# Jianxff/svo_pro_universal

Hardware: AMD Instinct MI355X
Metric: aligned patches/sec + ms/frame, EuRoC 640x480 mono, 1/2/4/8 MI355X (higher is better)
Workload: dtype f64

## Files before the change

### svo_pro_universal_amd/csrc/sparse_align.hip

```cpp
#include <atomic>
#include <cstdlib>
#include <cstring>

#include <type_traits>

#include "svoh_internal.h"
#include "svoh_device_utils.h"
#include "svoh_math.h"

#define SVOH_ALIGN_DRAIN(ctx) SVOH_HIP_TRY(ctx, svoh::align_drain(ctx))

namespace svoh {

static hipError_t align_drain(svoh_ctx* ctx);

static hipError_t align_side_setup(svoh_ctx* ctx, void* h, void* d, size_t bytes)
{
  if (ctx->align_copy_stream) return hipSuccess;
  hipError_t e = ctx->align_launches_since_drain ? align_drain(ctx) : hipSuccess;
  hipEvent_t* evs[] = { &ctx->ev_align_kernel[0], &ctx->ev_align_kernel[1], &ctx->ev_align_uploaded, &ctx->ev_align_delivered };
  for (hipEvent_t* ev : evs)
    if (e == hipSuccess && !*ev) e = hipEventCreateWithFlags(ev, hipEventDisableTiming);
  if (e == hipSuccess) e = hipStreamCreateWithFlags(&ctx->align_copy_stream, hipStreamNonBlocking);
  if (bytes > ((size_t)1 << 20)) bytes = (size_t)1 << 20;
// ... 59 lines not shown
  int32_t n_features;
  int32_t feat_off;
};

struct DevProblemDesc {
  int32_t n_cams, cam_begin;
  svoh_se3 T_init;
  double alpha_init, beta_init;
  svoh_align_prior prior;
};

struct AlignKernelArgs {
  const DevProblemDesc* problems;
  const DevCamDesc* cams;
  svoh_align_result* results;
  double* wpk;
  int64_t slots;
  uint8_t* wsel;
  uint8_t* wvis;
  svoh_align_options opt;
  int32_t lds_img_bytes;
  int32_t rig_build;
  int32_t latency_build;
  int32_t lds_two_per_cu;
  int32_t ws_lds_bytes;
  int32_t eval_level;
  double* eval_out;
  long long* stamps;
  int32_t n_problems;
  int32_t* queue;
  int32_t one_each;
  const svoh_align_gn_state* ext_state;
  int32_t raw_sums;
  int32_t cluster;
  double* xchg;
  unsigned int* bar;
#ifdef SVOH_TEST_HOOKS
  int32_t cluster_test_absent;
#endif
};

constexpr int kXchgStride = 64;

#ifdef SVOH_PHASE_STAMPS
#define SVOH_STAMP_DECL long long st_t0 = 0, st_acc[8] = {0, 0, 0, 0, 0, 0, 0, 0}; const long long st_begin = (long long)__builtin_amdgcn_s_memtime();
#define SVOH_STAMP_START() do { st_t0 = (long long)__builtin_amdgcn_s_memtime(); } while (0)
#define SVOH_STAMP_ADD(k) do { long long st_n = (long long)__builtin_amdgcn_s_memtime(); st_acc[k] += st_n - st_t0; st_t0 = st_n; } while (0)
// ... 146 lines not shown
    const ImgView<RLDS>& ref, const ImgView<CLDS>& cur, int ru, int rv, double rsu, double rsv, int cu, int cv,
    double csu, double csv, double one_plus_alpha, double beta, bool robust, float weight_scale,
    double (&mom)[AccLayout<D>::NMOM])
{
  constexpr int P = PW;
  constexpr int WB = P + 2;
  const double rwtl = (1.0 - rsu) * (1.0 - rsv), rwtr = rsu * (1.0 - rsv);
  const double rwbl = (1.0 - rsu) * rsv, rwbr = rsu * rsv;
  const double cwtl = ((1.0 - csu) * (1.0 - csv)) * one_plus_alpha, cwtr = (csu * (1.0 - csv)) * one_plus_alpha;
  const double cwbl = ((1.0 - csu) * csv) * one_plus_alpha, cwbr = (csu * csv) * one_plus_alpha;

  const int roff = rv * ref.pitch + ru;
  const int coff = cv * cur.pitch + cu;
  if constexpr (ZERO) {
#pragma unroll
    for (int k = 0; k < AccLayout<D>::NMOM; ++k) mom[k] = 0.0;
  }

  unsigned rawA[WB + 1], rawB[WB + 1];
  double it0[WB], it1[WB], it2[WB];
  unsigned curA[P + 1], curB[P + 1];
  PackedRow<WB + 1> pref_r;
  PackedRow<P + 1> pref_c;
  if constexpr (!RLDS) {
    PackedRow<WB + 1> r0, r1, r2;
    ref.template fetch<WB + 1>(roff, r0);
    ref.template fetch<WB + 1>(roff + ref.pitch, r1);
    ref.template fetch<WB + 1>(roff + 2 * ref.pitch, r2);
    ref.template fetch<WB + 1>(roff + 3 * ref.pitch, pref_r);
    if constexpr (!CLDS) {
      PackedRow<P + 1> c0;
      cur.template fetch<P + 1>(coff, c0);
      cur.template fetch<P + 1>(coff + cur.pitch, pref_c);
      ImgView<false>::unpack<P + 1>(c0, curB);
    }
    ImgView<false>::unpack<WB + 1>(r0, rawA);
    ImgView<false>::unpack<WB + 1>(r1, rawB);
#pragma unroll
    for (int i = 0; i < WB; ++i)
      it1[i] = rwtl * (double)rawA[i] + rwtr * (double)rawA[i + 1] + rwbl * (double)rawB[i] + rwbr * (double)rawB[i + 1];
    ImgView<false>::unpack<WB + 1>(r2, rawA);
  } else {
    ref.template row<WB + 1>(roff, rawA);
    ref.template row<WB + 1>(roff + ref.pitch, rawB);
#pragma unroll
    for (int i = 0; i < WB; ++i)
      it1[i] = rwtl * (double)rawA[i] + rwtr * (double)rawA[i + 1] + rwbl * (double)rawB[i] + rwbr * (double)rawB[i + 1];
    ref.template row<WB + 1>(roff + 2 * ref.pitch, rawA);
  }
#pragma unroll
  for (int i = 0; i < WB; ++i)
    it2[i] = rwtl * (double)rawB[i] + rwtr * (double)rawB[i + 1] + rwbl * (double)rawA[i] + rwbr * (double)rawA[i + 1];
  if constexpr (RLDS || CLDS) cur.template row<P + 1>(coff, curB);

  constexpr int kRowUnroll = GONLY ? 4 : (ROB ? 1 : (PH == 8 ? 4 : (D == 8 ? 1 : 2)));
#pragma unroll kRowUnroll
  for (int y = 0; y < PH; ++y) {
    const int rrow = roff + (y + 3) * ref.pitch;
    const int crow = coff + (y + 1) * cur.pitch;
#pragma unroll
    for (int i = 0; i < P + 1; ++i) curA[i] = curB[i];
    if constexpr (!RLDS && !CLDS) {
      ImgView<false>::unpack<WB + 1>(pref_r, rawB);
      ImgView<false>::unpack<P + 1>(pref_c, curB);
      if (y + 1 < PH) {
        ref.template fetch<WB + 1>(rrow + ref.pitch, pref_r);
        cur.template fetch<P + 1>(crow + cur.pitch, pref_c);
      }
      asm volatile("" ::: "memory");
    } else {
      ref.template row<WB + 1>(rrow, rawB);
      cur.template row<P + 1>(crow, curB);
    }
#pragma unroll
    for (int i = 0; i < WB; ++i) {
      it0[i] = it1[i];
      it1[i] = it2[i];
      it2[i] = rwtl * (double)rawA[i] + rwtr * (double)rawA[i + 1] + rwbl * (double)rawB[i] +
               rwbr * (double)rawB[i + 1];
    }
#pragma unroll
    for (int i = 0; i < WB + 1; ++i) rawA[i] = rawB[i];
#pragma unroll
    for (int x = 0; x < P; ++x) {
      const double ref_val = it1[x + 1];
      const double dx = it1[x + 2] - it1[x];
      const double dy = it2[x + 1] - it0[x + 1];
      const double res = fma(cwtl, (double)curA[x], fma(cwtr, (double)curA[x + 1], fma(cwbl, (double)curB[x], fma(cwbr, (double)curB[x + 1], beta - ref_val))));
      if constexpr (GONLY) {
        mom[3] += dx * res;
        mom[4] += dy * res;
        mom[5] += res * res;
// ... 373 lines not shown
    const double ru_tl = zu.y * scale - patch_center_wb;
    const double rv_tl = vs.x * scale - patch_center_wb;
    const int ru = (int)floor(ru_tl), rv = (int)floor(rv_tl);
    const double rsu = ru_tl - ru, rsv = rv_tl - rv;
    double mom[AccLayout<D>::NMOM];
    patch_rows_moments<P, LPP, D, LDS, LDS, GONLY, ROB>(ref, cur, ru, rv, rsu, rsv, cu, cv, csu, csv, r, one_plus_alpha, beta_d, robust,
                                                   weight_scale, mom);
#pragma unroll
    for (int k = 0; k < AccLayout<D>::NMOM; ++k)
      if (!GONLY || k == 3 || k == 4 || k == 5 || k == 13 || k == 14) asm volatile("" : "+v"(mom[k]));
    SVOH_PASS_STAMP(3);
    double ja[6], jb[6];
    jac_rows(jc, cm, dist_jac, X, scale, ja, jb);
    if constexpr (GONLY) accumulate_patch_gradient<D>(mom, ja, jb, est_alpha, est_beta, acc);
    else accumulate_patch<D>(mom, ja, jb, est_alpha, est_beta, acc);
#ifdef SVOH_PHASE_STAMPS
    asm volatile("" : "+v"(acc[0]), "+v"(acc[1]), "+v"(acc[2]));
#endif
    SVOH_PASS_STAMP(4);
  }
}

constexpr int kStageDoubles = 2 * kWsPairs * 128;
template <int P, int D, int NT, bool LDS, bool GONLY = false, bool ROB = false>
__device__ __forceinline__ void accumulate_camera_staged(
    const AlignKernelArgs& a, const CamPass& cd, const ImgView<LDS>& ref, const ImgView<LDS>& cur, int cw, int ch,
    const Rigid& Tcr, double scale, double one_plus_alpha, double beta_d, bool est_alpha, bool est_beta,
    bool robust, bool dist_jac, float weight_scale, int tid, double* stage, const double* jc,
    double (&acc)[GONLY ? D + 1 : AccLayout<D>::NACC], int& nvis, int& changed, int stride = NT)
{
  typedef const __attribute__((address_space(1))) void* gptr;
  typedef __attribute__((address_space(3))) void* lptr;
  const CamModel cm = load_camera(cd.cam);
  const double patch_center = (P - 1) / 2.0f;
  const double patch_center_wb = (P + 2 - 1) / 2.0f;
  const int lane = tid & 63;
  const int n = cd.n_features;
  const int n_round = (n + stride - 1) / stride * stride;
  auto request = [&](double* buf, int64_t gi) {
#pragma unroll
    for (int pr = 0; pr < kWsPairs; ++pr)
      __builtin_amdgcn_global_load_lds((gptr)ws_pair(a, pr, gi), (lptr)(buf + pr * 128), 16, 0, 0);
  };
  if (tid < n) request(stage, cd.feat_off + tid);
  int which = 0;
  for (int i = tid; i < n_round; i += stride, which ^= 1) {
    const int64_t gi = cd.feat_off + i;
    const bool in_range = i < n;
    double* buf = stage + which * (kWsPairs * 128);
// ... 15 lines not shown
        double u, v;
        project3(cm, Y, u, v);
        const double u_tl = u * scale - patch_center;
        const double v_tl = v * scale - patch_center;
        vis = !(u_tl < 0.0 || v_tl < 0.0 || u_tl + P + 2.0 >= cw || v_tl + P + 2.0 >= ch);
        vis = vis && u_tl == u_tl && v_tl == v_tl;
        if (vis) {
          const double fu = floor(u_tl), fv = floor(v_tl);
          cu = (int)fu; cv = (int)fv;
          csu = u_tl - cu; csv = v_tl - cv;
        }
      }
      if constexpr (GONLY) changed |= (int)((vs.y == 2.0) != vis);
      else {
        ws_pair(a, 2, gi)[1] = vis ? 2.0 : 1.0;
        if (a.eval_level >= 0) a.wvis[gi] = vis ? 1 : 0;
      }
      if (vis) {
        ++nvis;
        const double ru_tl = zu.y * scale - patch_center_wb;
        const double rv_tl = vs.x * scale - patch_center_wb;
        const int ru = (int)floor(ru_tl), rv = (int)floor(rv_tl);
        const double rsu = ru_tl - ru, rsv = rv_tl - rv;
        patch_moments<P, D, LDS, LDS, GONLY, ROB>(ref, cur, ru, rv, rsu, rsv, cu, cv, csu, csv, one_plus_alpha, beta_d,
                                                  robust, weight_scale, mom);
      }
    }
    if (vis) {
      if constexpr (LDS) {
#pragma unroll
        for (int k = 0; k < AccLayout<D>::NMOM; ++k)
          if (!GONLY || k == 3 || k == 4 || k == 5 || k == 13 || k == 14) asm volatile("" : "+v"(mom[k]));
      }

      asm volatile("" ::: "memory");
      const double2 xy2 = *reinterpret_cast<const double2*>(buf + 0 * 128 + lane * 2);
      const double z2 = buf[1 * 128 + lane * 2];
      const Vec3 X = { xy2.x, xy2.y, z2 };
      double ja[6], jb[6];
      jac_rows(jc, cm, dist_jac, X, scale, ja, jb);
      if constexpr (GONLY) accumulate_patch_gradient<D>(mom, ja, jb, est_alpha, est_beta, acc);
      else accumulate_patch<D>(mom, ja, jb, est_alpha, est_beta, acc);
    }
    __builtin_amdgcn_s_waitcnt(0xC07F);
  }
}

template <int NT>
__device__ __forceinline__ bool cluster_sum(const AlignKernelArgs& a, int prob, int share, unsigned& epoch, double* vals, int n,
                                            int tid, int* s_flag)
{
  const int G = a.cluster;
// ... 309 lines not shown
      s.Told = T; s.alpha_old = alpha; s.beta_old = beta;
      s.T = Tn; s.alpha = an; s.beta = bn;
      if (level_done) s.level_done = 1;
    }
    T = Tn; alpha = an; beta = bn;
  }
  SVOH_WAVE_STAMP(2);
  {
    const int c = lane < n_cams ? lane : 0;
    const Rigid Tcr = mul(mul(s.cam_cur_T_cam_imu[c], T), s.cam_ref_T_imu_cam[c]);
    if (lane < n_cams) s.Tcr[c] = Tcr;
    if (lane == 0) { s.alpha_f = (float)alpha; s.beta_f = (float)beta; }
  }
  SVOH_WAVE_STAMP(3);
}

template <int P, int NT, bool ILLUM, bool CLUSTER = false, bool ROBUST = false, int LPP = 1, bool LAT = false, bool RIG = false>
__global__ __launch_bounds__(NT, (NT == 256 ? (LAT ? 1 : 2) : 2))
void sparse_align_kernel(const AlignKernelArgs a)
{
  static_assert(!LAT || (NT == 256 && !CLUSTER && LPP == 1), "latency build: the 256-thread lane-per-patch geometry");
  static_assert(!RIG || (!CLUSTER && LPP == 1 && (LAT || NT == 512)), "rig build: the two lane-per-patch geometries of small launches");
  static_assert(LPP == 1 || (!CLUSTER && NT == 512 && LPP <= P), "rows geometry: 512 threads, no cluster mode");
  static_assert(NT == 256 || NT == 512, "workgroups of 256 or 512 threads");
  constexpr bool ROWS = LPP > 1;
  constexpr int D = ILLUM ? 8 : 6;
  constexpr int NACC = AccLayout<D>::NACC;
  constexpr int NW = NT / 64;

  constexpr bool STAGED = NT == 256 && !ROWS;
  constexpr bool kStageRegs = NT == 256 && !LAT && !CLUSTER && !ROWS;
  extern __shared__ __align__(16) unsigned char lds_img[];
  __shared__ __align__(16) double s_stage[STAGED ? NW * kStageDoubles : 2];
  __shared__ double s_jc[SVOH_MAX_CAMS][kJacConsts];
  __shared__ int s_lvl_off[SVOH_MAX_LEVELS];
  __shared__ double s_red[NW][NACC];
  static_assert(NACC <= 45, "g_sum is sized for the 8-parameter case");
  __shared__ double s_x[kXchgStride];
  __shared__ int s_cluster_ok;

  const int tid = threadIdx.x;
  const int lane = tid & 63, wave = tid >> 6;
  __shared__ int s_pbi;
  __shared__ StageItem s_stage_items[kMaxStageItems];
  for (;;) {
  __syncthreads();
  if (tid == 0) s_pbi = atomicAdd(a.queue, 1);
  __syncthreads();
  const int pbi = s_pbi;
  if (pbi >= a.n_problems) break;
#ifdef SVOH_TEST_HOOKS
  if (CLUSTER && a.cluster_test_absent && pbi % a.cluster == 1) continue;
#endif
  const DevProblemDesc& pb = a.problems[pbi];
// ... 103 lines not shown
      if (n_local * kWsPairs * 16 <= a.ws_lds_bytes) {
        ws.base = reinterpret_cast<double*>(lds_img + a.lds_img_bytes);
        ws.slots = n_local;
        ws.first = cams[0].feat_off;
      }
    }
  }
  {
    int my_sel = 0;
    const int patch_size_wb = P + 2;
    const double scale = 1.0f / (1 << opt.max_level);
    const double patch_center_wb = (patch_size_wb - 1) / 2.0f;
    for (int c = 0; c < n_cams; ++c) {
      const DevCamDesc& cd = cams[c];
      const int rows_minus_two = cd.ref[opt.max_level].h - 2;
      const int cols_minus_two = cd.ref[opt.max_level].w - 2;
      struct FeatIn { double pu, pv, pwx, pwy, pwz, fx, fy, fz; unsigned flag; };
      auto request = [&](int k, FeatIn& o) {
        o.flag = cd.flags[k];
        o.pu = cd.px[2 * k]; o.pv = cd.px[2 * k + 1];
        o.pwx = cd.pos_world[3 * k + 0]; o.pwy = cd.pos_world[3 * k + 1]; o.pwz = cd.pos_world[3 * k + 2];
        o.fx = cd.f[3 * k + 0]; o.fy = cd.f[3 * k + 1]; o.fz = cd.f[3 * k + 2];
      };
      constexpr int kBaseDepth = 4;
      for (int i0 = tid; i0 < cd.n_features; i0 += kBaseDepth * NT) {
        FeatIn in[kBaseDepth];
#pragma unroll
        for (int k = 0; k < kBaseDepth; ++k) {
          in[k] = FeatIn{ 0, 0, 0, 0, 0, 0, 0, 0, 0u };
          if (i0 + k * NT < cd.n_features) request(i0 + k * NT, in[k]);
        }
#pragma unroll
        for (int k = 0; k < kBaseDepth; ++k) {
          const int i = i0 + k * NT;
          if (i >= cd.n_features) break;
          const int gi = cd.feat_off + i;
          bool sel = in[k].flag != 0;
          const double pu = in[k].pu, pv = in[k].pv;
          const double pwx = in[k].pwx, pwy = in[k].pwy, pwz = in[k].pwz;
          const double fx_ = in[k].fx, fy_ = in[k].fy, fz_ = in[k].fz;
          if (sel) {
            const double u_tl = pu * scale - patch_center_wb;
            const double v_tl = pv * scale - patch_center_wb;
            const int u_tl_i = (int)floor(u_tl);
            const int v_tl_i = (int)floor(v_tl);
            sel = !(u_tl_i < 0 || v_tl_i < 0 || u_tl_i >= cols_minus_two - patch_size_wb ||
                    v_tl_i >= rows_minus_two - patch_size_wb);
          }
          a.wsel[gi] = sel ? 1 : 0;
          a.wvis[gi] = 0;
          if (!sel) *reinterpret_cast<double2*>(ws_pair(ws, 2, gi)) = make_double2(0.0, 0.0);
          if (sel) {
            const double dx = pwx - cd.ref_pos[0];
            const double dy = pwy - cd.ref_pos[1];
            const double dz = pwz - cd.ref_pos[2];
            const double depth = sqrt(dx * dx + dy * dy + dz * dz);
            const Vec3 X = { fx_ * depth, fy_ * depth, fz_ * depth };
            *reinterpret_cast<double2*>(ws_pair(ws, 0, gi)) = make_double2(X.x, X.y);
            *reinterpret_cast<double2*>(ws_pair(ws, 1, gi)) = make_double2(X.z, pu);
            *reinterpret_cast<double2*>(ws_pair(ws, 2, gi)) = make_double2(pv, 1.0);
            ++my_sel;
          }
        }
      }
    }
    if (my_sel) atomicAdd(&g_state.nsel, my_sel);
  }
  __syncthreads();
  SVOH_STAMP_ADD(0);
  constexpr bool cluster = CLUSTER;
  const int c_prob = cluster ? pbi / a.cluster : pbi;
  const int c_share = cluster ? pbi % a.cluster : 0;
  const int res_idx = cluster ? (c_share == 0 ? c_prob : a.n_problems / a.cluster + pbi) : pbi;
// ... 24 lines not shown
  const bool est_alpha = opt.estimate_illumination_gain != 0;
  const bool est_beta = opt.estimate_illumination_offset != 0;
  constexpr bool robust = ROBUST;
  const bool dist_jac = opt.use_distortion_jacobian != 0;
  const float weight_scale = (float)opt.weight_scale;

  constexpr int kLanesPerPatch = ROWS ? LPP : 1;
  bool side_by_side = false;
  if (RIG && n_cams >= 2) {
    int lanes_needed = 0;
    for (int c = 0; c < n_cams; ++c) lanes_needed += (cams[c].n_features * kLanesPerPatch + 63) & ~63;
    side_by_side = lanes_needed <= NT;
  }

  for (int level = level_hi; level >= level_lo; --level) {
    const double scale = 1.0f / (1 << level);
    int lvl_off = s_lvl_off[level];
    bool in_lds = lvl_off >= 0;
    if (!in_lds && level_bytes(level) <= a.lds_img_bytes) {
      __syncthreads();
      stage_level(level, 0);
      lvl_off = 0;
      in_lds = true;
    }
    __builtin_amdgcn_s_waitcnt(0x0F70);
    __syncthreads();
    if (tid == 0) {
      g_state.level_done = 0;
      for (int c = 0; c < n_cams; ++c)
        g_state.Tcr[c] = mul(mul(g_state.cam_cur_T_cam_imu[c], g_state.T), g_state.cam_ref_T_imu_cam[c]);
      g_state.alpha_f = (float)g_state.alpha; g_state.beta_f = (float)g_state.beta;
      g_state.Told = g_state.T; g_state.alpha_old = g_state.alpha; g_state.beta_old = g_state.beta;
    }
    __syncthreads();
    SVOH_STAMP_ADD(1);

    for (int iter = 0; iter < opt.max_iter; ++iter) {
      const double one_plus_alpha = uniform_f64(1.0 + (double)g_state.alpha_f);
      const double beta_d = uniform_f64((double)g_state.beta_f);
      bool light = !eval_mode && !robust && iter > 0;
      for (;;) {
        int nvis = 0, changed = 0;
        auto run_cameras = [&](auto gonly_tag, auto& acc_ref) {
          constexpr bool G = decltype(gonly_tag)::value;
          int off = lvl_off;
          int cam_base = 0;
          for (int c = 0; c < n_cams; ++c) {
            const DevCamDesc& cdg = cams[c];
            CamPass cd;
            cd.cam = cdg.cam; cd.n_features = cdg.n_features; cd.feat_off = cdg.feat_off;
            const DevImage& rim = cdg.ref[level];
            const DevImage& cim = cdg.cur[level];
            const Rigid Tcr = uniform_rigid(g_state.Tcr[c]);
            unsigned cam_stride = NT, cam_t = (unsigned)tid;
            if (RIG && side_by_side) {
              const int cam_width = (cd.n_features * kLanesPerPatch + 63) & ~63;
              cam_stride = (unsigned)cam_width;
              cam_t = (unsigned)(tid - cam_base);
              cam_base += cam_width;
            }
            if (in_lds) {
              ImgView<true> ref, cur;
              ref.p = (const __attribute__((address_space(3))) uint8_t*)(lds_img + off); ref.pitch = rim.w;
              off += ((rim.w * rim.h + 15) & ~15);
              cur.p = (const __attribute__((address_space(3))) uint8_t*)(lds_img + off); cur.pitch = cim.w;
              off += ((cim.w * cim.h + 15) & ~15);
              if constexpr (ROWS) {
                if (!RIG || cam_t < cam_stride)
                  accumulate_camera_rows<P, (ROWS ? LPP : 2), D, NT, true, G, ROBUST>(a, ws, cd, ref, cur, cim.w, cim.h, Tcr, scale, one_plus_alpha, beta_d,
                                                                            est_alpha, est_beta, robust, dist_jac, weight_scale, (int)cam_t, s_jc[c],
                                                                            acc_ref, nvis, changed, (int)cam_stride);
              } else if constexpr (STAGED) {
                if (!RIG || cam_t < cam_stride)
                  accumulate_camera_staged<P, D, NT, true, G, ROBUST>(a, cd, ref, cur, cim.w, cim.h, Tcr, scale, one_plus_alpha, beta_d,
                                                            est_alpha, est_beta, robust, dist_jac, weight_scale, (int)cam_t,
                                                            s_stage + wave * kStageDoubles, s_jc[c], acc_ref, nvis, changed, (int)cam_stride);
              }
              else if (!RIG || cam_t < cam_stride)
                accumulate_camera<P, D, NT, true, G, ROBUST>(a, ws, cd, ref, cur, cim.w, cim.h, Tcr, scale, one_plus_alpha, beta_d,
                                                     est_alpha, est_beta, robust, dist_jac, weight_scale, (int)cam_t, s_jc[c], acc_ref,
                                                     nvis, changed, (int)cam_stride);
            } else {
              ImgView<false> ref, cur;
              ref.p = rim.data; ref.pitch = rim.pitch;
// ... 174 lines not shown
  }
  gn_serial_step<P, D, ILLUM>(a, pb, cams, pb.n_cams, 0, level, iter, false, false);
  if (level < SVOH_MAX_LEVELS) {
    svoh_align_result& res = a.results[0];
    res.iters[level] = s.lvl_iters[level]; res.n_meas[level] = s.lvl_n_meas[level]; res.chi2[level] = s.lvl_chi2[level];
  }
  store_rigid(s.T, st->T_icur_iref);
  st->alpha = s.alpha; st->beta = s.beta;
  store_rigid(s.Told, st->T_old);
  st->alpha_old = s.alpha_old; st->beta_old = s.beta_old;
  for (int k = 0; k < 8; ++k) st->I_prior[k] = s.I_prior[k];
  st->chi2 = s_sum[NH + D] / (double)n_meas;
  st->n_meas = n_meas;
  st->stop = s.stop; st->level_done = s.level_done; st->status = s.status;
}

struct LaunchCfg { int nt; size_t lds; };

constexpr size_t kLdsPerCu = 163840;
template <int P, int NT, bool ILLUM, bool CLUSTER, bool ROBUST, int LPP = 1, bool LAT = false, bool RIG = false>
static hipError_t launch_one(hipStream_t st, int grid, size_t lds, AlignKernelArgs args, int32_t* lds_img_launched)
{
  auto kern = sparse_align_kernel<P, NT, ILLUM, CLUSTER, ROBUST, LPP, LAT, RIG>;
  if (NT == 256 && args.lds_two_per_cu) {
    static std::atomic<size_t> static_lds_cache{ 0 };
    size_t static_lds = static_lds_cache.load(std::memory_order_relaxed);
    if (static_lds == 0) {
      hipFuncAttributes attr;
      hipError_t ea = hipFuncGetAttributes(&attr, reinterpret_cast<const void*>(kern));
      if (ea != hipSuccess) return ea;
      static_lds = attr.sharedSizeBytes ? attr.sharedSizeBytes : 1;
      static_lds_cache.store(static_lds, std::memory_order_relaxed);
    }
    const size_t room = kLdsPerCu / 2 > static_lds ? (kLdsPerCu / 2 - static_lds) & ~(size_t)15 : 0;
    if (lds > room) {
      args.lds_img_bytes -= (int32_t)(lds - room);
      if (args.lds_img_bytes < 0) args.lds_img_bytes = 0;
      lds = room;
    }
  }
  hipError_t e = hipFuncSetAttribute(reinterpret_cast<const void*>(kern),
                                     hipFuncAttributeMaxDynamicSharedMemorySize, (int)lds);
  if (e != hipSuccess) return e;
  *lds_img_launched = args.lds_img_bytes;
  hipLaunchKernelGGL(kern, dim3(grid), dim3(NT), lds, st, args);
  return hipGetLastError();
}

template <int P, bool ILLUM, bool ROBUST>
static hipError_t launch_nt(hipStream_t st, int nt, int lpp, int grid, size_t lds, const AlignKernelArgs& args, int32_t* lds_img_launched)
{
  if (args.cluster > 1) return launch_one<P, 256, ILLUM, true, ROBUST>(st, grid, lds, args, lds_img_launched);
  if (nt == 256) {
    if (args.latency_build) return args.rig_build ? launch_one<P, 256, ILLUM, false, ROBUST, 1, true, true>(st, grid, lds, args, lds_img_launched)
                                                  : launch_one<P, 256, ILLUM, false, ROBUST, 1, true>(st, grid, lds, args, lds_img_launched);
    return launch_one<P, 256, ILLUM, false, ROBUST>(st, grid, lds, args, lds_img_launched);
  }
  if (lpp <= 1 && args.rig_build) return launch_one<P, 512, ILLUM, false, ROBUST, 1, false, true>(st, grid, lds, args, lds_img_launched);
  switch (lpp) {
    case 2: return launch_one<P, 512, ILLUM, false, ROBUST, 2>(st, grid, lds, args, lds_img_launched);
    case 4: return launch_one<P, 512, ILLUM, false, ROBUST, 4>(st, grid, lds, args, lds_img_launched);
    case 8: if constexpr (P == 8) return launch_one<P, 512, ILLUM, false, ROBUST, 8>(st, grid, lds, args, lds_img_launched);
    default: return launch_one<P, 512, ILLUM, false, ROBUST>(st, grid, lds, args, lds_img_launched);
  }
}

constexpr int kWsLdsMaxFeatures = 340;
constexpr int kClusterMinFeatures = 512;
constexpr int kClusterMaxWorkgroups = 32;
constexpr int kClusterMaxProblems = 64;

static int validate_options(svoh_ctx* ctx, const svoh_align_options* o)
{
  SVOH_REQUIRE(ctx, o != nullptr, "options is NULL");
  if (o->patch_size != 4 && o->patch_size != 8)
    return set_error(ctx, SVOH_ERR_UNSUPPORTED, "patch_size %d not built (4 and 8 are)", o->patch_size);
  SVOH_REQUIRE(ctx, o->max_level >= o->min_level && o->min_level >= 0 && o->max_level < SVOH_MAX_LEVELS,
               "bad level range");
  SVOH_REQUIRE(ctx, o->max_iter >= 1, "max_iter must be >= 1");
  return SVOH_OK;
}

struct SplitArgs {
  const svoh_align_gn_state* ext_state = nullptr;
  double* sums_out = nullptr;
  const double* sums_in = nullptr;
  svoh_align_gn_state* state = nullptr;
  int iter = 0;
  bool update = false;
  int n_shares = 1;
};

struct AlignGeometry {
  int cluster_g = 0;
  int nt = 256;
  int rows = 1;
  bool latency = false;
  bool rig = false;
  int32_t key() const { return (1 << 30) | (cluster_g & 0xff) | ((nt == 512 ? 1 : 0) << 8) | ((rows & 0xf) << 9) | ((latency ? 1 : 0) << 13) | ((rig ? 1 : 0) << 14); }
  static bool from_key(int32_t k, AlignGeometry* g)
  {
    if (!(k & (1 << 30)) || (k & ~((1 << 30) | 0x7fff))) return false;
    g->cluster_g = k & 0xff; g->nt = (k >> 8) & 1 ? 512 : 256; g->rows = (k >> 9) & 0xf; g->latency = (k >> 13) & 1; g->rig = (k >> 14) & 1;
    return (g->rows == 1 || g->rows == 2 || g->rows == 4 || g->rows == 8) && g->cluster_g != 1 && g->cluster_g <= kClusterMaxWorkgroups;
  }
};

static int decide_cluster(const svoh_ctx* ctx, int n_problems, const svoh_align_problem* problems)
{
  if (n_problems > kClusterMaxProblems || ctx->align_no_cluster) return 0;
  int64_t nf_min = INT64_MAX, nf_max = 0;
  for (int p = 0; p < n_problems; ++p) {
    int64_t nf = 0;
    if (problems[p].n_cams >= 1 && problems[p].n_cams <= SVOH_MAX_CAMS)
      for (int c = 0; c < problems[p].n_cams; ++c) nf += problems[p].cams[c].n_features > 0 ? problems[p].cams[c].n_features : 0;
    nf_min = nf < nf_min ? nf : nf_min;
    nf_max = nf > nf_max ? nf : nf_max;
  }
  int g = SvohKnobs::or_default(ctx->knobs.align_cluster, -1);
  const bool worth = nf_min >= kClusterMinFeatures && (n_problems <= 16 || nf_min >= 3000);
  auto workgroups_for = [](int64_t nf) {
    if (nf < 875) return 3;
    if (nf < 1250) return 4;
    if (nf < 1750) return 6;
    if (nf < 5000) return 8;
    if (nf < 7000) return 12;
// ... 17 lines not shown
    z->have_rig = true;
    int lanes = 0;
    for (int c = 0; c < pb.n_cams; ++c) lanes += (pb.cams[c].n_features + 63) & ~63;
    z->rig_wants_512 = z->rig_wants_512 || (lanes > 256 && lanes <= 512);
  }
}

static AlignGeometry decide_geometry(const svoh_ctx* ctx, const svoh_align_options* opt, int n_desc, int cluster_g, const LaunchShape& z)
{
  AlignGeometry g;
  const bool cluster = cluster_g >= 2;
  g.cluster_g = cluster ? cluster_g : 0;
  int nt = (n_desc >= ctx->num_cus) ? 256 : 512;
  if (z.max_feat_per_problem <= 256) nt = 256;
  if (!cluster && n_desc < ctx->num_cus && z.rig_wants_512) nt = 512;
  int rows = 1;
  if (!cluster && n_desc < ctx->num_cus) {
    while (rows * 2 <= opt->patch_size && rows * 2 <= 8 && (int64_t)z.max_feat_per_problem * rows * 2 <= 256) rows *= 2;
  }
  rows = SvohKnobs::or_default(ctx->knobs.align_rows, rows);
  if (rows != 2 && rows != 4 && rows != 8) rows = 1;
  if (rows > opt->patch_size || cluster) rows = 1;
  if (rows > 1) nt = 512;
  nt = SvohKnobs::or_default(ctx->knobs.align_threads, nt);
  if (cluster) nt = 256;
  if (nt != 256 && nt != 512) nt = 256;
  if (nt == 256) rows = 1;
  g.nt = nt; g.rows = rows;
  g.latency = nt == 256 && !cluster && n_desc < ctx->num_cus && SvohKnobs::or_default(ctx->knobs.align_latency_build, 1) != 0;
  g.rig = !cluster && n_desc < ctx->num_cus && z.have_rig && (g.latency || nt == 512);
  return g;
}

static bool shared_class_geometry(const svoh_ctx* ctx, const svoh_align_problem& pb, AlignGeometry* g)
{
  if (!ctx->align_shared_classes || ctx->align_no_cluster) return false;
  if (pb.n_cams < 1 || pb.n_cams > SVOH_MAX_CAMS) return false;
  int64_t nf = 0;
  for (int c = 0; c < pb.n_cams; ++c) nf += pb.cams[c].n_features > 0 ? pb.cams[c].n_features : 0;
  if (nf >= kClusterMinFeatures) return false;
  *g = AlignGeometry();
  g->cluster_g = 0; g->nt = 512; g->rows = 1; g->latency = false; g->rig = pb.n_cams >= 2;
  return true;
}

static AlignGeometry geometry_of_single(const svoh_ctx* ctx, const svoh_align_options* opt, const svoh_align_problem& pb)
{
  AlignGeometry shared;
  if (shared_class_geometry(ctx, pb, &shared)) return shared;
  const int g = decide_cluster(ctx, 1, &pb);
// ... 188 lines not shown
          if ((int)n > pos_jobs_max_n) pos_jobs_max_n = (int)n;
          up_off += (n * 4 + 63) & ~(size_t)63;
        }
        const uint8_t* dv = share_base[c];
        dc.px = reinterpret_cast<const double*>(dv) + 2 * lo;
        dc.f = reinterpret_cast<const double*>(dv + n * 16) + 3 * lo;
        dc.pos_world = reinterpret_cast<const double*>(dv + n * 40) + 3 * lo;
        dc.flags = dv + n * 64 + lo;
      }
    }
  }
  const PosFromSeedsJob* pos_jobs_device = nullptr;
  if (!pos_jobs.empty()) {
    memcpy(hup + up_off, pos_jobs.data(), sizeof(PosFromSeedsJob) * pos_jobs.size());
    pos_jobs_device = reinterpret_cast<const PosFromSeedsJob*>(dup + up_off);
    up_off += (sizeof(PosFromSeedsJob) * pos_jobs.size() + 63) & ~(size_t)63;
  }
  const int side_knob = ctx->knobs.align_side_copies;
  const bool side_kind = n_desc >= ctx->num_cus && !cluster && !split && !forced && eval_level < 0 &&
                         (side_knob == kKnobUnset ? up_base + up_off > ((size_t)1 << 20) : side_knob != 0);
  if (side_kind) SVOH_HIP_TRY(ctx, align_side_setup(ctx, h_desc.ptr, d_desc.ptr, up_base + up_off));
  const AlignGeometry geo = forced ? *forced : decide_geometry(ctx, opt, n_desc, cluster ? S : 0, shape);
  const int overlap_knob = ctx->knobs.align_overlap;
  const bool lane_kind = n_desc >= ctx->num_cus && geo.nt == 256 && !geo.latency && !cluster && !split && !forced && eval_level < 0 && n_pos_jobs == 0 &&
                         (overlap_knob == kKnobUnset || overlap_knob != 0);
  if (lane_kind) SVOH_HIP_TRY(ctx, align_lane_setup(ctx, h_desc.ptr, d_desc.ptr, up_base + up_off));
  const size_t feat_bytes = feat_slots * (kWsPairs * 16 + 2) + 256;
  {
    const bool to_lane1 = lane_kind && ctx->align_chain && ctx->align_launches_since_drain >= 1 && ctx->align_last_lane == 0;
    DevBuffer& ws = to_lane1 ? ctx->d_feat_lane1 : ctx->d_feat;
    if (ws.ptr && feat_bytes > ws.cap && ctx->align_launches_since_drain >= 1 && ctx->align_lane_stream && ctx->align_lane1_launches) {
      SVOH_ALIGN_DRAIN(ctx);
      SVOH_HIP_TRY(ctx, ws.reserve(feat_bytes));
    }
  }
  const bool overlapped = lane_kind && ctx->align_chain && ctx->align_launches_since_drain >= 1;
  const int lane = overlapped ? (ctx->align_last_lane ^ 1) : 0;
  DevBuffer& d_feat = lane ? ctx->d_feat_lane1 : ctx->d_feat;
  SVOH_HIP_TRY(ctx, d_feat.reserve(feat_bytes));
  const hipStream_t prev_stream = ctx->align_stream_of(ctx->align_last_lane);
  if (lane) {
    if (ctx->align_lane1_wants_front) {
      SVOH_HIP_TRY(ctx, hipStreamWaitEvent(ctx->align_lane_stream, ctx->ev_align_front, 0));
      ctx->align_lane1_wants_front = false;
    }
  } else if (!overlapped) {
    SVOH_ALIGN_JOIN(ctx);
// ... 80 lines not shown
    if (S == 1) args.eval_out = split->sums_out;
    args.raw_sums = 1;
  }
  if (split && split->update) {
    const bool illum_u = opt->estimate_illumination_gain || opt->estimate_illumination_offset;
    if (opt->patch_size == 4) {
      if (illum_u) hipLaunchKernelGGL((align_gn_update_kernel<4, true>), dim3(1), dim3(64), 0, ctx->stream, args, split->sums_in, split->state, eval_level, split->iter);
      else hipLaunchKernelGGL((align_gn_update_kernel<4, false>), dim3(1), dim3(64), 0, ctx->stream, args, split->sums_in, split->state, eval_level, split->iter);
    } else {
      if (illum_u) hipLaunchKernelGGL((align_gn_update_kernel<8, true>), dim3(1), dim3(64), 0, ctx->stream, args, split->sums_in, split->state, eval_level, split->iter);
      else hipLaunchKernelGGL((align_gn_update_kernel<8, false>), dim3(1), dim3(64), 0, ctx->stream, args, split->sums_in, split->state, eval_level, split->iter);
    }
    const hipError_t eu = hipGetLastError();
    if (eu != hipSuccess) return set_error(ctx, SVOH_ERR_HIP, "gn_update launch failed: %s", hipGetErrorString(eu));
    return SVOH_OK;
  }
  args.queue = reinterpret_cast<int32_t*>(static_cast<uint8_t*>(d_desc.ptr) + ctl_off);
#ifdef SVOH_PHASE_STAMPS
  SVOH_HIP_TRY(ctx, ctx->d_scratch0.reserve(sizeof(long long) * 20 * (size_t)n_problems));
  args.stamps = static_cast<long long*>(ctx->d_scratch0.ptr);
#endif

  const int nt = geo.nt, rows = geo.rows;
  size_t lds = (nt == 256) ? 52224 : 78 * 1024;
  args.latency_build = geo.latency ? 1 : 0;
  args.rig_build = geo.rig ? 1 : 0;
  args.lds_two_per_cu = (nt == 256 && !cluster && ctx->knobs.align_lds == kKnobUnset && ctx->knobs.align_wg_per_cu == kKnobUnset) ? 1 : 0;
  lds = (size_t)SvohKnobs::or_default(ctx->knobs.align_lds, (int)lds) & ~(size_t)15;
  const size_t lds_cap = (nt == 256) ? 163840 - 32768 : 153856;
  if (lds > lds_cap) lds = lds_cap;
  args.ws_lds_bytes = 0;
  if (nt == 512 && !cluster && max_feat_per_problem <= kWsLdsMaxFeatures && lds >= (size_t)kWsLdsMaxFeatures * kWsPairs * 16 + 4096) {
    args.ws_lds_bytes = ((max_feat_per_problem > 0 ? max_feat_per_problem : 1) * kWsPairs * 16 + 15) & ~15;
  }
  args.lds_img_bytes = (int32_t)(lds - (size_t)args.ws_lds_bytes);

  const bool illum = opt->estimate_illumination_gain || opt->estimate_illumination_offset;
  int grid = ctx->num_cus * SvohKnobs::or_default(ctx->knobs.align_wg_per_cu, nt == 256 ? 2 : 1);
  if (grid > n_desc || grid <= 0) grid = n_desc;
  if (cluster) grid = n_desc;
  args.one_each = 0;
  hipError_t e;
  const bool timed = ctx->timing_on();
  const int ev_slot = (int)(ctx->align_timed_launches % svoh_ctx::kAlignEventRing);
  if (timed) SVOH_HIP_TRY(ctx, hipEventRecord(ctx->ev_align_start[ev_slot], ks));
  const bool robust = opt->robustification != 0;
  int32_t lds_img_launched = 0;
#ifdef SVOH_DEV_ONLY_PLAIN
  if (robust || illum) return set_error(ctx, SVOH_ERR_UNSUPPORTED, "development build: plain kernels only");
  e = opt->patch_size == 4 ? launch_nt<4, false, false>(ks, nt, rows, grid, lds, args, &lds_img_launched)
                           : launch_nt<8, false, false>(ks, nt, rows, grid, lds, args, &lds_img_launched);
#else
  if (opt->patch_size == 4) {
    if (robust) e = illum ? launch_nt<4, true, true>(ks, nt, rows, grid, lds, args, &lds_img_launched) : launch_nt<4, false, true>(ks, nt, rows, grid, lds, args, &lds_img_launched);
    else e = illum ? launch_nt<4, true, false>(ks, nt, rows, grid, lds, args, &lds_img_launched) : launch_nt<4, false, false>(ks, nt, rows, grid, lds, args, &lds_img_launched);
  } else {
    if (robust) e = illum ? launch_nt<8, true, true>(ks, nt, rows, grid, lds, args, &lds_img_launched) : launch_nt<8, false, true>(ks, nt, rows, grid, lds, args, &lds_img_launched);
    else e = illum ? launch_nt<8, true, false>(ks, nt, rows, grid, lds, args, &lds_img_launched) : launch_nt<8, false, false>(ks, nt, rows, grid, lds, args, &lds_img_launched);
  }
#endif
  if (e != hipSuccess)
// ... 321 lines not shown
```

### svo_pro_universal_amd/frontend.py

```python
import ctypes as C

import numpy as np

from . import _capi as capi


class SvohError(RuntimeError):
    def __init__(self, code, msg):
        RuntimeError.__init__(self, "svoh error %d: %s" % (code, msg))
        self.code = code


def _se3(T):
    s = capi.svoh_se3()
    v = T.as7() if hasattr(T, "as7") else np.asarray(T, dtype=np.float64)
    for i in range(4):
        s.q[i] = float(v[i])
    for i in range(3):
        s.t[i] = float(v[4 + i])
    return s


def _camera(cam):
    c = capi.svoh_camera()
# ... 162 lines not shown
    def sparse_align(self, opt, problems):
        n = len(problems)
        res = (capi.svoh_align_result * n)()
        self._check(self.lib.svoh_sparse_align_batch(self.h, C.byref(opt), n, problems, res))
        return res

    def sparse_align_enqueue(self, opt, problems):
        self._check(self.lib.svoh_sparse_align_enqueue(self.h, C.byref(opt), len(problems), problems))

    def sparse_align_fetch(self, n):
        res = (capi.svoh_align_result * n)()
        self._check(self.lib.svoh_sparse_align_fetch(self.h, n, res))
        return res

    def sparse_align_fetch_all(self, n_total):
        res = (capi.svoh_align_result * n_total)()
        self._check(self.lib.svoh_sparse_align_fetch_all(self.h, n_total, res))
        return res

    def last_align_launch(self):
        key, grid, n_desc = C.c_int32(), C.c_int32(), C.c_int32()
        self._check(self.lib.svoh_sparse_align_last_launch_info(self.h, C.byref(key), C.byref(grid), C.byref(n_desc)))
        k = key.value
        return dict(key=k, cluster_g=k & 0xff, nt=512 if (k >> 8) & 1 else 256, rows=(k >> 9) & 0xf,
                    latency=bool((k >> 13) & 1), rig=bool((k >> 14) & 1), grid=grid.value, n_desc=n_desc.value)

    def last_align_lane(self):
        lane, lanes, n1 = C.c_int32(), C.c_int32(), C.c_uint64()
        self._check(self.lib.svoh_sparse_align_last_launch_lane(self.h, C.byref(lane), C.byref(lanes), C.byref(n1)))
        return dict(lane=lane.value, lanes=lanes.value, lane1_launches=int(n1.value))

    def last_align_launch_lds(self):
        n = C.c_int32()
        self._check(self.lib.svoh_sparse_align_last_launch_lds(self.h, C.byref(n)))
        return n.value

    def sparse_align_evaluate(self, opt, problem, level):
        H = np.zeros(64)
        g = np.zeros(8)
        chi2, nm, nsel = C.c_double(), C.c_int32(), C.c_int32()
        ntot = sum(problem.cams[i].n_features for i in range(problem.n_cams))
        vis = np.zeros(max(1, ntot), np.uint8)
        self._check(self.lib.svoh_sparse_align_evaluate(self.h, C.byref(opt), C.byref(problem), level,
                                                        H.ctypes.data, g.ctypes.data, C.byref(chi2), C.byref(nm),
                                                        vis.ctypes.data, C.byref(nsel)))
        return H.reshape(8, 8).T.copy(), g, chi2.value, nm.value, vis[:nsel.value].copy()

# ... 429 lines not shown
```

Baseline: 2.463 billion.

## Add 128-thread sparse-align geometry with ref-only LDS staging for large batches

Adds a 128-thread workgroup variant of the staged sparse-align kernel, picked for patch size 4 when there are many problems per CU. It runs four workgroups per CU and sizes LDS to a quarter share. When a level does not fit fully in LDS, only the reference image is staged there and the current image is read from global with row prefetching, through a new mixed ref-LDS/cur-global path in the patch moment loop. It also skips the wsel/wvis writes outside eval mode and deepens base-feature batching for this geometry. The aim is more resident workgroups and more latency hiding, at the cost of less LDS per workgroup, more global image reads, and another kernel instantiation.

New measurement: 2.581 billion, median of 6. +4.8%, better.

```diff
diff --git a/svo_pro_universal_amd/csrc/sparse_align.hip b/svo_pro_universal_amd/csrc/sparse_align.hip
--- a/svo_pro_universal_amd/csrc/sparse_align.hip
+++ b/svo_pro_universal_amd/csrc/sparse_align.hip
@@ -105,7 +105,7 @@
   int32_t lds_img_bytes;
   int32_t rig_build;
   int32_t latency_build;
-  int32_t lds_two_per_cu;
+  int32_t lds_wg_per_cu;
   int32_t ws_lds_bytes;
   int32_t eval_level;
   double* eval_out;
@@ -298,6 +298,11 @@
   unsigned curA[P + 1], curB[P + 1];
   PackedRow<WB + 1> pref_r;
   PackedRow<P + 1> pref_c;
+  PackedRow<P + 1> c0_mixed;
+  if constexpr (RLDS && !CLDS) {
+    cur.template fetch<P + 1>(coff, c0_mixed);
+    cur.template fetch<P + 1>(coff + cur.pitch, pref_c);
+  }
   if constexpr (!RLDS) {
     PackedRow<WB + 1> r0, r1, r2;
     ref.template fetch<WB + 1>(roff, r0);
@@ -327,7 +332,8 @@
 #pragma unroll
   for (int i = 0; i < WB; ++i)
     it2[i] = rwtl * (double)rawB[i] + rwtr * (double)rawB[i + 1] + rwbl * (double)rawA[i] + rwbr * (double)rawA[i + 1];
-  if constexpr (RLDS || CLDS) cur.template row<P + 1>(coff, curB);
+  if constexpr (RLDS && !CLDS) ImgView<false>::unpack<P + 1>(c0_mixed, curB);
+  else if constexpr (CLDS) cur.template row<P + 1>(coff, curB);
 
   constexpr int kRowUnroll = GONLY ? 4 : (ROB ? 1 : (PH == 8 ? 4 : (D == 8 ? 1 : 2)));
 #pragma unroll kRowUnroll
@@ -344,6 +350,11 @@
         cur.template fetch<P + 1>(crow + cur.pitch, pref_c);
       }
       asm volatile("" ::: "memory");
+    } else if constexpr (RLDS && !CLDS) {
+      ImgView<false>::unpack<P + 1>(pref_c, curB);
+      if (y + 1 < PH) cur.template fetch<P + 1>(crow + cur.pitch, pref_c);
+      asm volatile("" ::: "memory");
+      ref.template row<WB + 1>(rrow, rawB);
     } else {
       ref.template row<WB + 1>(rrow, rawB);
       cur.template row<P + 1>(crow, curB);
@@ -763,9 +774,9 @@
 }
 
 constexpr int kStageDoubles = 2 * kWsPairs * 128;
-template <int P, int D, int NT, bool LDS, bool GONLY = false, bool ROB = false>
+template <int P, int D, int NT, bool LDS, bool GONLY = false, bool ROB = false, bool CLDS = LDS>
 __device__ __forceinline__ void accumulate_camera_staged(
-    const AlignKernelArgs& a, const CamPass& cd, const ImgView<LDS>& ref, const ImgView<LDS>& cur, int cw, int ch,
+    const AlignKernelArgs& a, const CamPass& cd, const ImgView<LDS>& ref, const ImgView<CLDS>& cur, int cw, int ch,
     const Rigid& Tcr, double scale, double one_plus_alpha, double beta_d, bool est_alpha, bool est_beta,
     bool robust, bool dist_jac, float weight_scale, int tid, double* stage, const double* jc,
     double (&acc)[GONLY ? D + 1 : AccLayout<D>::NACC], int& nvis, int& changed, int stride = NT)
@@ -827,12 +838,12 @@
         const double rv_tl = vs.x * scale - patch_center_wb;
         const int ru = (int)floor(ru_tl), rv = (int)floor(rv_tl);
         const double rsu = ru_tl - ru, rsv = rv_tl - rv;
-        patch_moments<P, D, LDS, LDS, GONLY, ROB>(ref, cur, ru, rv, rsu, rsv, cu, cv, csu, csv, one_plus_alpha, beta_d,
-                                                  robust, weight_scale, mom);
+        patch_moments<P, D, LDS, CLDS, GONLY, ROB>(ref, cur, ru, rv, rsu, rsv, cu, cv, csu, csv, one_plus_alpha, beta_d,
+                                                   robust, weight_scale, mom);
       }
     }
     if (vis) {
-      if constexpr (LDS) {
+      if constexpr (LDS && CLDS) {
 #pragma unroll
         for (int k = 0; k < AccLayout<D>::NMOM; ++k)
           if (!GONLY || k == 3 || k == 4 || k == 5 || k == 13 || k == 14) asm volatile("" : "+v"(mom[k]));
@@ -1188,14 +1199,16 @@
   static_assert(!LAT || (NT == 256 && !CLUSTER && LPP == 1), "latency build: the 256-thread lane-per-patch geometry");
   static_assert(!RIG || (!CLUSTER && LPP == 1 && (LAT || NT == 512)), "rig build: the two lane-per-patch geometries of small launches");
   static_assert(LPP == 1 || (!CLUSTER && NT == 512 && LPP <= P), "rows geometry: 512 threads, no cluster mode");
-  static_assert(NT == 256 || NT == 512, "workgroups of 256 or 512 threads");
+  static_assert(NT == 128 || NT == 256 || NT == 512, "workgroups of 128, 256 or 512 threads");
+  static_assert(NT != 128 || (!CLUSTER && !LAT && !RIG && LPP == 1), "128 threads: the batch geometry only");
   constexpr bool ROWS = LPP > 1;
   constexpr int D = ILLUM ? 8 : 6;
   constexpr int NACC = AccLayout<D>::NACC;
   constexpr int NW = NT / 64;
 
-  constexpr bool STAGED = NT == 256 && !ROWS;
-  constexpr bool kStageRegs = NT == 256 && !LAT && !CLUSTER && !ROWS;
+  constexpr bool STAGED = (NT == 256 || NT == 128) && !ROWS;
+  constexpr bool kStageRegs = (NT == 256 || NT == 128) && !LAT && !CLUSTER && !ROWS;
+  constexpr bool kHalfLevel = NT == 128;
   extern __shared__ __align__(16) unsigned char lds_img[];
   __shared__ __align__(16) double s_stage[STAGED ? NW * kStageDoubles : 2];
   __shared__ double s_jc[SVOH_MAX_CAMS][kJacConsts];
@@ -1345,7 +1358,7 @@
         o.pwx = cd.pos_world[3 * k + 0]; o.pwy = cd.pos_world[3 * k + 1]; o.pwz = cd.pos_world[3 * k + 2];
         o.fx = cd.f[3 * k + 0]; o.fy = cd.f[3 * k + 1]; o.fz = cd.f[3 * k + 2];
       };
-      constexpr int kBaseDepth = 4;
+      constexpr int kBaseDepth = NT == 128 ? 8 : 4;
       for (int i0 = tid; i0 < cd.n_features; i0 += kBaseDepth * NT) {
         FeatIn in[kBaseDepth];
 #pragma unroll
@@ -1370,8 +1383,7 @@
             sel = !(u_tl_i < 0 || v_tl_i < 0 || u_tl_i >= cols_minus_two - patch_size_wb ||
                     v_tl_i >= rows_minus_two - patch_size_wb);
           }
-          a.wsel[gi] = sel ? 1 : 0;
-          a.wvis[gi] = 0;
+          if (eval_mode) { a.wsel[gi] = sel ? 1 : 0; a.wvis[gi] = 0; }
           if (!sel) *reinterpret_cast<double2*>(ws_pair(ws, 2, gi)) = make_double2(0.0, 0.0);
           if (sel) {
             const double dx = pwx - cd.ref_pos[0];
@@ -1442,6 +1454,19 @@
       stage_level(level, 0);
       lvl_off = 0;
       in_lds = true;
+    }
+    bool half_lds = false;
+    if constexpr (kHalfLevel) {
+      if (!in_lds && n_cams == 1) {
+        const DevImage& him = cams[0].ref[level];
+        if (((him.w * him.h + 15) & ~15) <= a.lds_img_bytes) {
+          __syncthreads();
+          DevImage none = him;
+          none.w = none.h = none.pitch = 0;
+          stage_image_pair<NT, kStageRegs>(lds_img, him, lds_img, none, tid);
+          half_lds = true;
+        }
+      }
     }
     __builtin_amdgcn_s_waitcnt(0x0F70);
     __syncthreads();
@@ -1479,7 +1504,17 @@
               cam_t = (unsigned)(tid - cam_base);
               cam_base += cam_width;
             }
-            if (in_lds) {
+            if (kHalfLevel && half_lds) {
+              if constexpr (kHalfLevel) {
+                ImgView<true> ref;
+                ImgView<false> cur;
+                ref.p = (const __attribute__((address_space(3))) uint8_t*)lds_img; ref.pitch = rim.w;
+                cur.p = cim.data; cur.pitch = cim.pitch;
+                accumulate_camera_staged<P, D, NT, true, G, ROBUST, false>(a, cd, ref, cur, cim.w, cim.h, Tcr, scale, one_plus_alpha, beta_d,
+                                                                                   est_alpha, est_beta, robust, dist_jac, weight_scale, (int)cam_t,
+                                                                                   s_stage + wave * kStageDoubles, s_jc[c], acc_ref, nvis, changed, (int)cam_stride);
+              }
+            } else if (in_lds) {
               ImgView<true> ref, cur;
               ref.p = (const __attribute__((address_space(3))) uint8_t*)(lds_img + off); ref.pitch = rim.w;
               off += ((rim.w * rim.h + 15) & ~15);
@@ -1700,7 +1735,8 @@
 static hipError_t launch_one(hipStream_t st, int grid, size_t lds, AlignKernelArgs args, int32_t* lds_img_launched)
 {
   auto kern = sparse_align_kernel<P, NT, ILLUM, CLUSTER, ROBUST, LPP, LAT, RIG>;
-  if (NT == 256 && args.lds_two_per_cu) {
+  if ((NT == 256 || NT == 128) && args.lds_wg_per_cu > 0) {
+    const size_t share = kLdsPerCu / (size_t)args.lds_wg_per_cu;
     static std::atomic<size_t> static_lds_cache{ 0 };
     size_t static_lds = static_lds_cache.load(std::memory_order_relaxed);
     if (static_lds == 0) {
@@ -1710,7 +1746,7 @@
       static_lds = attr.sharedSizeBytes ? attr.sharedSizeBytes : 1;
       static_lds_cache.store(static_lds, std::memory_order_relaxed);
     }
-    const size_t room = kLdsPerCu / 2 > static_lds ? (kLdsPerCu / 2 - static_lds) & ~(size_t)15 : 0;
+    const size_t room = share > static_lds ? (share - static_lds) & ~(size_t)15 : 0;
     if (lds > room) {
       args.lds_img_bytes -= (int32_t)(lds - room);
       if (args.lds_img_bytes < 0) args.lds_img_bytes = 0;
@@ -1729,6 +1765,7 @@
 static hipError_t launch_nt(hipStream_t st, int nt, int lpp, int grid, size_t lds, const AlignKernelArgs& args, int32_t* lds_img_launched)
 {
   if (args.cluster > 1) return launch_one<P, 256, ILLUM, true, ROBUST>(st, grid, lds, args, lds_img_launched);
+  if (nt == 128) return launch_one<P, 128, ILLUM, false, ROBUST>(st, grid, lds, args, lds_img_launched);
   if (nt == 256) {
     if (args.latency_build) return args.rig_build ? launch_one<P, 256, ILLUM, false, ROBUST, 1, true, true>(st, grid, lds, args, lds_img_launched)
                                                   : launch_one<P, 256, ILLUM, false, ROBUST, 1, true>(st, grid, lds, args, lds_img_launched);
@@ -1747,6 +1784,7 @@
 constexpr int kClusterMinFeatures = 512;
 constexpr int kClusterMaxWorkgroups = 32;
 constexpr int kClusterMaxProblems = 64;
+constexpr int kAlign128MinRounds = 4;
 
 static int validate_options(svoh_ctx* ctx, const svoh_align_options* o)
 {
@@ -1775,11 +1813,12 @@
   int rows = 1;
   bool latency = false;
   bool rig = false;
-  int32_t key() const { return (1 << 30) | (cluster_g & 0xff) | ((nt == 512 ? 1 : 0) << 8) | ((rows & 0xf) << 9) | ((latency ? 1 : 0) << 13) | ((rig ? 1 : 0) << 14); }
+  int32_t key() const { return (1 << 30) | (cluster_g & 0xff) | ((nt == 512 ? 1 : 0) << 8) | ((rows & 0xf) << 9) | ((latency ? 1 : 0) << 13) | ((rig ? 1 : 0) << 14) | ((nt == 128 ? 1 : 0) << 15); }
   static bool from_key(int32_t k, AlignGeometry* g)
   {
-    if (!(k & (1 << 30)) || (k & ~((1 << 30) | 0x7fff))) return false;
-    g->cluster_g = k & 0xff; g->nt = (k >> 8) & 1 ? 512 : 256; g->rows = (k >> 9) & 0xf; g->latency = (k >> 13) & 1; g->rig = (k >> 14) & 1;
+    if (!(k & (1 << 30)) || (k & ~((1 << 30) | 0xffff))) return false;
+    if (((k >> 15) & 1) && (k & 0x7fff) != 0x0200) return false;
+    g->cluster_g = k & 0xff; g->nt = (k >> 15) & 1 ? 128 : (k >> 8) & 1 ? 512 : 256; g->rows = (k >> 9) & 0xf; g->latency = (k >> 13) & 1; g->rig = (k >> 14) & 1;
     return (g->rows == 1 || g->rows == 2 || g->rows == 4 || g->rows == 8) && g->cluster_g != 1 && g->cluster_g <= kClusterMaxWorkgroups;
   }
 };
@@ -1843,10 +1882,13 @@
   if (rows != 2 && rows != 4 && rows != 8) rows = 1;
   if (rows > opt->patch_size || cluster) rows = 1;
   if (rows > 1) nt = 512;
+  const bool can_128 = !cluster && !z.have_rig;
+  if (can_128 && nt == 256 && opt->patch_size == 4 && n_desc >= kAlign128MinRounds * 4 * ctx->num_cus) nt = 128;
   nt = SvohKnobs::or_default(ctx->knobs.align_threads, nt);
   if (cluster) nt = 256;
-  if (nt != 256 && nt != 512) nt = 256;
-  if (nt == 256) rows = 1;
+  if (nt == 128 && !can_128) nt = 256;
+  if (nt != 128 && nt != 256 && nt != 512) nt = 256;
+  if (nt != 512) rows = 1;
   g.nt = nt; g.rows = rows;
   g.latency = nt == 256 && !cluster && n_desc < ctx->num_cus && SvohKnobs::or_default(ctx->knobs.align_latency_build, 1) != 0;
   g.rig = !cluster && n_desc < ctx->num_cus && z.have_rig && (g.latency || nt == 512);
@@ -2081,7 +2123,7 @@
   if (side_kind) SVOH_HIP_TRY(ctx, align_side_setup(ctx, h_desc.ptr, d_desc.ptr, up_base + up_off));
   const AlignGeometry geo = forced ? *forced : decide_geometry(ctx, opt, n_desc, cluster ? S : 0, shape);
   const int overlap_knob = ctx->knobs.align_overlap;
-  const bool lane_kind = n_desc >= ctx->num_cus && geo.nt == 256 && !geo.latency && !cluster && !split && !forced && eval_level < 0 && n_pos_jobs == 0 &&
+  const bool lane_kind = n_desc >= ctx->num_cus && (geo.nt == 256 || geo.nt == 128) && !geo.latency && !cluster && !split && !forced && eval_level < 0 && n_pos_jobs == 0 &&
                          (overlap_knob == kKnobUnset || overlap_knob != 0);
   if (lane_kind) SVOH_HIP_TRY(ctx, align_lane_setup(ctx, h_desc.ptr, d_desc.ptr, up_base + up_off));
   const size_t feat_bytes = feat_slots * (kWsPairs * 16 + 2) + 256;
@@ -2208,12 +2250,12 @@
 #endif
 
   const int nt = geo.nt, rows = geo.rows;
-  size_t lds = (nt == 256) ? 52224 : 78 * 1024;
+  size_t lds = (nt == 256) ? 52224 : (nt == 128) ? 24576 : 78 * 1024;
   args.latency_build = geo.latency ? 1 : 0;
   args.rig_build = geo.rig ? 1 : 0;
-  args.lds_two_per_cu = (nt == 256 && !cluster && ctx->knobs.align_lds == kKnobUnset && ctx->knobs.align_wg_per_cu == kKnobUnset) ? 1 : 0;
+  args.lds_wg_per_cu = (!cluster && ctx->knobs.align_lds == kKnobUnset && ctx->knobs.align_wg_per_cu == kKnobUnset) ? (nt == 256 ? 2 : nt == 128 ? 4 : 0) : 0;
   lds = (size_t)SvohKnobs::or_default(ctx->knobs.align_lds, (int)lds) & ~(size_t)15;
-  const size_t lds_cap = (nt == 256) ? 163840 - 32768 : 153856;
+  const size_t lds_cap = (nt == 256 || nt == 128) ? 163840 - 32768 : 153856;
   if (lds > lds_cap) lds = lds_cap;
   args.ws_lds_bytes = 0;
   if (nt == 512 && !cluster && max_feat_per_problem <= kWsLdsMaxFeatures && lds >= (size_t)kWsLdsMaxFeatures * kWsPairs * 16 + 4096) {
@@ -2222,7 +2264,7 @@
   args.lds_img_bytes = (int32_t)(lds - (size_t)args.ws_lds_bytes);
 
   const bool illum = opt->estimate_illumination_gain || opt->estimate_illumination_offset;
-  int grid = ctx->num_cus * SvohKnobs::or_default(ctx->knobs.align_wg_per_cu, nt == 256 ? 2 : 1);
+  int grid = ctx->num_cus * SvohKnobs::or_default(ctx->knobs.align_wg_per_cu, nt == 256 ? 2 : nt == 128 ? 4 : 1);
   if (grid > n_desc || grid <= 0) grid = n_desc;
   if (cluster) grid = n_desc;
   args.one_each = 0;
diff --git a/svo_pro_universal_amd/frontend.py b/svo_pro_universal_amd/frontend.py
--- a/svo_pro_universal_amd/frontend.py
+++ b/svo_pro_universal_amd/frontend.py
@@ -208,7 +208,7 @@
         key, grid, n_desc = C.c_int32(), C.c_int32(), C.c_int32()
         self._check(self.lib.svoh_sparse_align_last_launch_info(self.h, C.byref(key), C.byref(grid), C.byref(n_desc)))
         k = key.value
-        return dict(key=k, cluster_g=k & 0xff, nt=512 if (k >> 8) & 1 else 256, rows=(k >> 9) & 0xf,
+        return dict(key=k, cluster_g=k & 0xff, nt=128 if (k >> 15) & 1 else 512 if (k >> 8) & 1 else 256, rows=(k >> 9) & 0xf,
                     latency=bool((k >> 13) & 1), rig=bool((k >> 14) & 1), grid=grid.value, n_desc=n_desc.value)
 
     def last_align_lane(self):
```
